# jmschrei/PyPore

Measured on AMD Instinct MI355X. Metric: Msamples/sec segmented (SpeedyStatSplit, 10^8-sample trace); %HBM roofline, higher is better.
Workload: dtype int32/f64 (exact integer block sums of fp32 or int16 samples; decisions in fp64)

## Files before the change

### pypore_amd/csrc/poreseg.hip

```cpp
#include <hip/hip_runtime.h>

#include <algorithm>
#include <atomic>
#include <chrono>
#include <complex>
#include <cmath>
#include <cstdarg>
#include <cstdio>
#include <cstdlib>
#include <cstring>
#include <initializer_list>
#include <condition_variable>
#include <mutex>
#include <string>
#include <thread>
#include <tuple>
#include <type_traits>
#include <vector>

#include "poreseg.h"
#include "seg_device.hpp"
#include "seg_align.hpp"
#include "seg_pairwise.hpp"
#include "seg_trf.hpp"
// ... 41 lines not shown

struct HostBuf : NoCopy {
    void *p = nullptr;
    size_t cap = 0;
    ~HostBuf() { release(); }
    hipError_t reserve(size_t bytes)
    {
        if (bytes <= cap) return hipSuccess;
        release();
        size_t want = std::max(bytes, cap + cap / 2);
        hipError_t e = hipHostMalloc(&p, want, hipHostMallocDefault);
        if (e == hipSuccess) { cap = want; g_live_bytes += cap; }
        return e;
    }
    void release() { if (p) { (void)hipHostFree(p); g_live_bytes -= cap; } p = nullptr; cap = 0; }
    template <class T> T *as() { return static_cast<T *>(p); }
};

struct Event : NoCopy {
    hipEvent_t e = nullptr;
    ~Event() { if (e) (void)hipEventDestroy(e); }
    operator hipEvent_t() const { return e; }
};

struct Stream : NoCopy {
    hipStream_t s = nullptr;
    bool own = false;
    ~Stream() { if (own && s) (void)hipStreamDestroy(s); }
    operator hipStream_t() const { return s; }
};

}

enum : int { SC_NO_LA = 1, SC_NO_UPLOAD = 2, SC_ALL = 3 };
constexpr int LA_KEEP = 16;
struct ps_ctx {
    int device = 0;
    int n_cu = 0;
    Stream stream;
    Event ev[10];
    Event ev_front[2];
    ~ps_ctx() { (void)hipSetDevice(device); if (stream.s) (void)hipStreamSynchronize(stream.s); }
    std::string err;
    int64_t tile_len = 0, halo = 0;
    int mode = MODE_FAST, spine_nt = 512, tree_nt = 256;
    int lds_max_samples = 0;
    int rep_eval = 1, rep_stage = 1, rep_sum = 1;
    uint8_t *d_is_spine = nullptr;
    int prune = 1;
    double wide_quantum = 0;
    int wide_skip = 0;
    int wide_mode = 0;
    int tree_mw = 0;
    int upload_by_kernel = 1;
    int k0_waves = 0;
    float noise_k = 0.1f;
    int k0_admit = 0;
    int k0_sets = 2;
    bool chain_held = false;
    unsigned long long chain_ticket = 0;
    bool defer_sync = false;
    int scan_lds_pad = 0;
    int k0_unaligned = 1;
    int single_pass = 1;
    int gather_fused = 1;
    int download_by_kernel = 1;
    int debug = 0;
// ... 36 lines not shown
        long long budget = 2ll << 30;
    } trf;
    DevBuf ev_info_tr;
    DevBuf blk_cls, cls_mm;
    DevBuf pre_c;
    struct { DevBuf tab, pre, tmp, stack, cnt, off; } ss;
    struct { DevBuf tab, tab2, mask, cnt, excl, off1, off2, hits, pair_off, keep, kept, y, len, span_off; } sp;
    struct {
        DevBuf log;
        int64_t cap = 65536, hdr_cap = -1;
        int64_t seen = -1, call_cap = 0;
        std::vector<int64_t> ev_start, ev_len;
    } nt;
    struct {
        DevBuf model, off, bp, last, flags;
        std::vector<char> blob;
        long long bp_budget = 512ll << 20;
        DevBuf fmat, acc, skip;
        DevBuf pmax;
        DevBuf samp;
        long long fb_budget = 4ll << 30;
        bool expect_lds = true;
    } hmm;
    int stitch_host = 0;
    DevBuf ev_len, det_counts, det_tics, det_cand;
    DevBuf bridges, bmeta, tile_i32, sp_off, spine_items, asm_hdr, ev_first_tile;
    DevBuf bridge_ext, ext_slot, ext_list;
    DevBuf lat_state, lat_seam, lat_res;
    unsigned lat_tag_next = 1;
    unsigned lat_tag_base = 0;
    int lat_help = 1;
    int bridge_budget = BR_MAX;
    int bridge_ext_on = 1;
    int short_chain = SC_ALL;
    int shared_n = 0;
    int hw_queues = 0;
    int pool_patience = BR_PATIENCE_POOL;
    int la_keep = 0;
    bool la_now = false;
    bool small_clean = false;
    bool small_clean_in = false;
    HostBuf h_hdr;
    DevBuf spine_jobs, spine_scratch, spine_dense, spine_meta, tree_jobs, tree_scratch, tree_spill, tree_defer, screen_acc,
        tree_counts, items, item_pos, first_item, ev_off, bounds_off, small;
    HostBuf h_meta, h_dense, h_small, h_up;
    int timing = 1;
    double ms[8] = {0, 0, 0, 0, 0, 0, 0, 0};
    int64_t counters[20] = {0, 0, 0, 0, 0, 0, 0, 0, 0, 0, 0, 0, 0, 0, -1, -1, 0, 0, 0, 0};
    bool screen_ran = false;
};

namespace {

int fail(ps_ctx *ctx, int code, const char *fmt, ...)
{
    if (ctx) {
        char buf[512];
        va_list ap;
        va_start(ap, fmt);
        vsnprintf(buf, sizeof buf, fmt, ap);
        va_end(ap);
        ctx->err = buf;
    }
    return code;
}

#define HIP_TRY(ctx, expr)                                                                        \
    do {                                                                                          \
        hipError_t e_ = (expr);                                                                   \
        if (e_ != hipSuccess)                                                                     \
            return fail(ctx, PS_ERR_HIP, "%s failed: %s (%s:%d)", #expr, hipGetErrorString(e_), __FILE__, __LINE__); \
    } while (0)

struct FrontStream { std::mutex mu; hipStream_t s = nullptr; };
FrontStream g_front[16];
FrontStream *front_for(ps_ctx *ctx)
{
    if (ctx->device < 0 || ctx->device >= 16) return nullptr;
    FrontStream *f = &g_front[ctx->device];
    std::lock_guard<std::mutex> lk(f->mu);
    if (!f->s) {
// ... 387 lines not shown
    return j;
}

int find_in(const TileList &t, int32_t pos)
{
    if (pos == t.start) return -1;
    auto it = std::lower_bound(t.a.begin(), t.a.end(), pos, [](const Anchor &x, int32_t v) { return x.pos < v; });
    if (it != t.a.end() && it->pos == pos) return static_cast<int>(it - t.a.begin());
    return -2;
}

}

namespace {
constexpr int RC_FALLBACK = 1;
constexpr int RC_WIDE = 2;
int finish_batch(ps_ctx *ctx, const DevCfg &cfg, size_t n_tj, int64_t n_items, int32_t n_ev,
                        int32_t *d_bounds, int64_t cap, int64_t *h_bounds_off, ps_segstat *d_stats,
                        std::chrono::steady_clock::time_point t_begin, const AsmHeader *d_hdr = nullptr,
                        AsmHeader *hdr_out = nullptr, bool wide_check = false)
{
    int rc;
    const size_t evb = (static_cast<size_t>(n_ev) + 1) * sizeof(int64_t);
    SmallLayout *sm = ctx->small.as<SmallLayout>();
    if (ctx->timing >= 2) HIP_TRY(ctx, hipEventRecord(ctx->ev[2], ctx->stream));
    if (n_tj) {
        const unsigned g = static_cast<unsigned>(std::min<size_t>(n_tj, 0x7fffffff));
        if (int lrc = launch_subtrees(ctx, cfg, g, sm, n_tj, d_hdr)) return lrc;
    }
    if (ctx->timing >= 2) HIP_TRY(ctx, hipEventRecord(ctx->ev[3], ctx->stream));
    const bool fused = d_hdr != nullptr && ctx->gather_fused;
    const bool one_copy = ctx->bounds_off.p == ctx->small.as<char>() + sizeof(SmallLayout);
    int dl_clear = 0;
    if (fused) {
        const int64_t blocks = (n_items >> GS_LOG) + 1;
        const unsigned gg = static_cast<unsigned>(std::max<int64_t>(1, std::min<int64_t>(blocks, 1024)));
        hipLaunchKernelGGL(gather_scan_kernel, dim3(gg), dim3(1 << GS_LOG), 0, ctx->stream, ctx->items.as<Item>(),
                           ctx->tree_jobs.as<TreeJob>(), ctx->tree_counts.as<int32_t>(), ctx->tree_scratch.as<int32_t>(),
                           static_cast<long long>(n_items), d_bounds, cap, ctx->d_is_spine, d_hdr, ctx->first_item.as<int64_t>(),
                           n_ev, ctx->bounds_off.as<int64_t>());
        HIP_TRY(ctx, hipGetLastError());
    } else {
    hipLaunchKernelGGL(item_scan_kernel, dim3(1), dim3(1024), 0, ctx->stream, ctx->items.as<Item>(),
                       ctx->tree_counts.as<int32_t>(), n_items, ctx->item_pos.as<int64_t>(), d_hdr,
                       ctx->first_item.as<int64_t>(), n_ev, ctx->bounds_off.as<int64_t>());
    HIP_TRY(ctx, hipGetLastError());
    }
    if (n_items && !fused) {
        const unsigned gg = static_cast<unsigned>(d_hdr ? std::min<int64_t>(n_items, 16384) : n_items);
        hipLaunchKernelGGL(gather_kernel, dim3(gg), dim3(64), 0, ctx->stream,
                           ctx->items.as<Item>(), ctx->tree_jobs.as<TreeJob>(), ctx->tree_counts.as<int32_t>(),
                           ctx->tree_scratch.as<int32_t>(), ctx->item_pos.as<int64_t>(), n_items, d_bounds, cap, ctx->d_is_spine,
                           d_hdr);
        HIP_TRY(ctx, hipGetLastError());
    }
    const bool stats_from_digest = d_stats != nullptr && cfg.bsum != nullptr && cfg.blk_mm != nullptr;
    if (stats_from_digest) {
        const int64_t scap = cap + n_ev;
        const unsigned sg = static_cast<unsigned>(std::min<int64_t>(std::max<int64_t>(scap, 1), 8192));
        by_dtype(cfg.dtype, [&](auto dt) {
            hipLaunchKernelGGL(segstat_bs_kernel<dt()>, dim3(sg), dim3(64), 0, ctx->stream, cfg, ctx->ev_off.as<int64_t>(),
                               ctx->ev_len.as<int64_t>(), n_ev, d_bounds, ctx->bounds_off.as<int64_t>(), d_stats, scap,
                               reinterpret_cast<unsigned *>(&sm->status), d_hdr);
        });
        HIP_TRY(ctx, hipGetLastError());
        if (ctx->timing >= 2) HIP_TRY(ctx, hipEventRecord(ctx->ev[4], ctx->stream));
    }
    if (one_copy) {
        HIP_TRY(ctx, ctx->h_small.reserve(sizeof(SmallLayout) + evb));
        void *h_dev = nullptr;
        if (ctx->download_by_kernel && hipHostGetDevicePointer(&h_dev, ctx->h_small.p, 0) != hipSuccess) { h_dev = nullptr; (void)hipGetLastError(); }
        if (h_dev) {
            static_assert(sizeof(SmallLayout) % 8 == 0, "the status block is copied in 8-byte words");
            const long long nw = static_cast<long long>((sizeof(SmallLayout) + evb) / 8);
            if (fused && d_stats == nullptr && ctx->screen_ran && (ctx->short_chain & SC_NO_UPLOAD)) dl_clear = static_cast<int>(sizeof(SmallLayout) / 8);
            hipLaunchKernelGGL(download_kernel, dim3(static_cast<unsigned>(std::min<long long>((nw + 255) / 256, 64))), dim3(256), 0, ctx->stream,
                               ctx->small.as<unsigned long long>(), static_cast<unsigned long long *>(h_dev), nw, dl_clear, &sm->hdr.fail);
            HIP_TRY(ctx, hipGetLastError());
        } else {
            HIP_TRY(ctx, hipMemcpyAsync(ctx->h_small.p, ctx->small.p, sizeof(SmallLayout) + evb, hipMemcpyDeviceToHost, ctx->stream));
        }
    } else {
        HIP_TRY(ctx, ctx->h_meta.reserve(evb));
        HIP_TRY(ctx, hipMemcpyAsync(ctx->h_meta.p, ctx->bounds_off.p, evb, hipMemcpyDeviceToHost, ctx->stream));
        HIP_TRY(ctx, hipMemcpyAsync(ctx->h_small.p, ctx->small.p, sizeof(SmallLayout), hipMemcpyDeviceToHost, ctx->stream));
    }
    if (ctx->timing >= 1) HIP_TRY(ctx, hipEventRecord(ctx->ev[9], ctx->stream));
    HIP_TRY(ctx, hipStreamSynchronize(ctx->stream));
    {
        float seq = 0;
        if (ctx->timing >= 1 && hipEventElapsedTime(&seq, ctx->ev[8], ctx->ev[9]) == hipSuccess) ctx->ms[7] = seq;
    }
    std::memcpy(h_bounds_off, one_copy ? ctx->h_small.as<char>() + sizeof(SmallLayout) : ctx->h_meta.as<char>(), evb);
    const SmallLayout hs = *ctx->h_small.as<SmallLayout>();
    if (wide_check && (static_cast<unsigned>(hs.status) & ST_WIDE_RANGE)) return RC_WIDE;
    rc = check_status(ctx, static_cast<unsigned>(hs.status));
    if (rc) return rc;
    if (d_hdr) {
        const AsmHeader hd = hs.hdr;
        if (hdr_out) *hdr_out = hd;
        if (hd.fail) {
            if (ctx->debug) {
                const size_t nt = static_cast<size_t>(ctx->counters[2]);
                std::vector<int4> bm(nt), mt(nt);
                std::vector<SpineJob> jb(nt);
                if (nt && hipMemcpy(bm.data(), ctx->bmeta.p, nt * sizeof(int4), hipMemcpyDeviceToHost) == hipSuccess &&
                    hipMemcpy(mt.data(), ctx->spine_meta.p, nt * sizeof(int4), hipMemcpyDeviceToHost) == hipSuccess &&
                    hipMemcpy(jb.data(), ctx->spine_jobs.p, nt * sizeof(SpineJob), hipMemcpyDeviceToHost) == hipSuccess) {
// ... 415 lines not shown
    if (front) {
        HIP_TRY(ctx, hipEventRecord(ctx->ev_front[1], fs));
        front_lock.unlock();
        HIP_TRY(ctx, hipStreamWaitEvent(ctx->stream, ctx->ev_front[1], 0));
    }
    if (nj) {
        const unsigned g = static_cast<unsigned>(nj);
        int lrc;
        if (wide) lrc = launch_scans_bs<DT_WIDE>(ctx, cfg, g, sm);
        else if (use_bs) lrc = launch_scans_bs<0>(ctx, cfg, g, sm);
        else {
            lrc = launch_spine_nt(ctx, cfg, g, sm, true);
            if (lrc) return lrc;
            if (ctx->timing >= 2) HIP_TRY(ctx, hipEventRecord(ctx->ev[6], ctx->stream));
            lrc = by_nt<256, 512>(ctx->spine_nt, [&](auto nt) {
                return by_dtype(cfg.dtype, [&](auto dt) { return launch_bridge<decltype(nt)::value, dt()>(ctx, cfg, g, sm); });
            });
        }
        if (lrc) return lrc;
    }
    if (ctx->timing >= 2) HIP_TRY(ctx, hipEventRecord(ctx->ev[1], ctx->stream));
    int *ti = ctx->tile_i32.as<int>();
    const size_t njp = std::max<size_t>(1, nj);
    const size_t tile_lds = (nj + 1) * sizeof(long long) + 4 * nj * sizeof(int);
    const int use_lds = tile_lds <= 150 * 1024;
    if (use_lds)
        HIP_TRY(ctx, set_dyn_lds(ctx, reinterpret_cast<const void *>(assemble_tiles_kernel), static_cast<int>(tile_lds)));
    AsmHeader hd = {};
    int rc = PS_OK;
    int64_t items_cap = max_items;
    int slots_used = 0, ext_stride = EXT_MAX;
    const bool no_la = nj && no_look_ahead(ctx, cfg);
    bool la_done = false, stride_set = false;
    for (int round = 0;; ++round) {
        hipLaunchKernelGGL(assemble_tiles_kernel, dim3(1), dim3(1024), use_lds ? tile_lds : 0, ctx->stream,
                           static_cast<int>(nj), ctx->spine_meta.as<int4>(), ctx->bmeta.as<int4>(),
                           ctx->ev_first_tile.as<int64_t>(), n_ev, ti, ti + njp, ti + 2 * njp, ti + 3 * njp,
                           ctx->sp_off.as<long long>(), ctx->first_item.as<int64_t>(), ctx->asm_hdr.as<AsmHeader>(),
                           static_cast<long long>(items_cap), use_lds, reinterpret_cast<const unsigned *>(&sm->status));
        HIP_TRY(ctx, hipGetLastError());
        const AsmHeader *d_hdr = ctx->asm_hdr.as<AsmHeader>();
        if (items_cap > 0) {
            const unsigned ag = static_cast<unsigned>(std::min<int64_t>((items_cap + 255) / 256, 2048));
            hipLaunchKernelGGL(assemble_items_kernel, dim3(ag), dim3(256), 0,
                               ctx->stream, ctx->spine_jobs.as<SpineJob>(), static_cast<int>(nj), ctx->spine_meta.as<int4>(),
                               ctx->spine_scratch.as<int2>(), ctx->bridges.as<int2>(), ti + 3 * njp,
                               ctx->sp_off.as<long long>(), static_cast<long long>(items_cap), mw, W, ctx->tree_jobs.as<TreeJob>(),
                               ctx->items.as<Item>(), ctx->tree_counts.as<int32_t>(), d_hdr, cfg.bsum != nullptr ? cfg.ev_info : nullptr,
                               ctx->bridge_ext.as<int2>(), ctx->ext_slot.as<int>(), ext_stride);
            HIP_TRY(ctx, hipGetLastError());
        }
        if (ctx->timing >= 2 && round == 0) HIP_TRY(ctx, hipEventRecord(ctx->ev[5], ctx->stream));
        rc = finish_batch(ctx, cfg, static_cast<size_t>(items_cap), items_cap, n_ev, d_bounds, cap, h_bounds_off, d_stats, t_begin,
                          d_hdr, &hd, use_bs);
        if (rc != RC_FALLBACK || !use_bs || !nj || round == EXT_ROUNDS + (la_done ? 1 : 0) || !ctx->bridge_ext_on) break;
        HIP_TRY(ctx, ctx->h_meta.reserve(2 * nj * sizeof(int4)));
        int4 *h_bm = ctx->h_meta.as<int4>(), *h_mt = h_bm + nj;
        HIP_TRY(ctx, hipMemcpyAsync(h_bm, ctx->bmeta.p, nj * sizeof(int4), hipMemcpyDeviceToHost, ctx->stream));
        HIP_TRY(ctx, hipMemcpyAsync(h_mt, ctx->spine_meta.p, nj * sizeof(int4), hipMemcpyDeviceToHost, ctx->stream));
        HIP_TRY(ctx, hipStreamSynchronize(ctx->stream));
        if (no_la && !la_done) {
            int64_t n_def = 0;
            for (size_t g = 0; g < nj; ++g) n_def += h_bm[g].w == BR_DEFER || h_bm[g].w == BR_DEFER_REACHED;
            if (n_def) {
                if (ctx->debug) fprintf(stderr, "[poreseg] look-ahead kernel behind the stitch: %lld deferred seams\n", static_cast<long long>(n_def));
                HIP_TRY(ctx, hipMemsetAsync(&sm->hdr, 0, sizeof(AsmHeader), ctx->stream));
                if (ctx->tree_screen) HIP_TRY(ctx, hipMemsetAsync(&sm->tree_defer[0], 0, sizeof sm->tree_defer[0], ctx->stream));
                if (int lrc = by_dtype(cfg.dtype, [&](auto dt) { return launch_bridge_la<dt()>(ctx, cfg, static_cast<unsigned>(nj), sm); })) return lrc;
                la_done = true;
                ctx->la_keep = LA_KEEP;
                ctx->counters[4] += n_def;
                ctx->counters[18] += n_def;
                continue;
            }
        }
        std::vector<int> list;
        bool hopeless = false;
        if (!stride_set) {
            size_t n_fail = 0;
            for (size_t g = 0; g < nj; ++g) n_fail += h_bm[g].w == BR_FAIL_REACHED || (h_bm[g].w == BR_FAIL && h_bm[g].x == ctx->bridge_budget);
            ext_stride = n_fail <= static_cast<size_t>(EXT_SLOTS) ? EXT_MAX : EXT_MAX_MANY;
            stride_set = true;
        }
// ... 228 lines not shown
    else if (n == "scan_bs") ctx->scan_bs = value != 0;
    else if (n == "near_tie_log" && value >= 0 && value <= (int64_t(1) << 30)) ctx->nt.cap = value;
    else if (n == "groups") ctx->groups = value != 0;
    else if (n == "tree_par") ctx->tree_par = value != 0;
    else if (n == "k0_waves" && value >= 0 && value <= 16) ctx->k0_waves = static_cast<int>(value);
    else if (n == "k0_shared") ctx->k0_shared = value != 0;
    else if (n == "k0_admit" && value >= 0) ctx->k0_admit = static_cast<int>(value);
    else if (n == "bridge_ext" && (value == 0 || value == 1)) ctx->bridge_ext_on = static_cast<int>(value);
    else if (n == "lat_help" && value >= 0 && value <= 2) ctx->lat_help = static_cast<int>(value);
    else if (n == "shared_device" && value >= 0 && value <= 4096) {
        ps_pool_plan_t plan;
        if (pool_plan(static_cast<int>(value), ctx->hw_queues > 0 ? ctx->hw_queues : process_hw_queues(), &plan) != PS_OK)
            return fail(ctx, PS_ERR_ARG, "shared_device: no plan for %lld contexts", static_cast<long long>(value));
        ctx->shared_n = static_cast<int>(value);
        ctx->la_keep = 0;
        ctx->k0_waves = plan.k0_waves;
        ctx->lat_help = plan.lat_help;
        ctx->k0_admit = plan.k0_admit;
    }
    else if (n == "hw_queues" && value >= 0 && value <= HW_QUEUES_MAX) ctx->hw_queues = static_cast<int>(value);
    else if (n == "hmm_bp_budget" && value >= 1) ctx->hmm.bp_budget = value;
    else if (n == "hmm_fb_budget" && value >= 1) ctx->hmm.fb_budget = value;
    else if (n == "pairwise_budget" && value >= 1) ctx->pw.budget = value;
    else if (n == "trf_budget" && value >= 1) ctx->trf.budget = value;
    else if (n == "hmm_expect_lds") ctx->hmm.expect_lds = value != 0;
    else if (n == "single_pass") ctx->single_pass = value != 0;
    else if (n == "gather_fused") ctx->gather_fused = value != 0;
    else if (n == "download_by_kernel") ctx->download_by_kernel = value != 0;
    else if (n == "debug") ctx->debug = value != 0;
    else if (n == "k0_unaligned") ctx->k0_unaligned = value != 0 ? k0_unaligned_probe(ctx->device, ctx->stream) : 0;
    else if (n == "slots_pct" && value >= 1 && value <= 100) ctx->slots_pct = static_cast<int>(value);
    else if (n == "tree_jobs_per_wave" && value >= 0 && value <= 1024) ctx->tree_jobs_per_wave = static_cast<int>(value);
    else if (n == "tree_screen") ctx->tree_screen = value != 0;
    else if (n == "short_chain" && value >= 0 && value <= 3) {
        static const int bits[4] = {0, SC_ALL, SC_NO_LA, SC_NO_UPLOAD};
        if (ctx->short_chain != bits[value]) ctx->small_clean = false;
        ctx->short_chain = bits[value];
    }
    else if (n == "bridge_patience" && value >= 1 && value <= 4096) { ctx->pool_patience = static_cast<int>(value); ctx->la_keep = 0; }
    else if (n == "noise_k_ppm" && value >= 0) ctx->noise_k = static_cast<float>(static_cast<double>(value) * 1.0e-6);
#ifdef PS_DIAG
    else if (n == "dbg_phase" && value >= 0 && value <= 2) ctx->dbg_phase = static_cast<int>(value);
    else if (n == "dbg_k0_nogrp") ctx->dbg_k0_nogrp = value != 0;
    else if (n == "cu_mask" && ctx->stream.own)
        return diag_mask_stream(ctx, &ctx->stream.s, static_cast<int>(value & 0xfff), static_cast<int>((value >> 12) & 0xfff),
                                static_cast<int>((value >> 24) & 0xff), ((value >> 32) & 1) != 0);
    else if (n == "k0_sets" && value >= 2 && value <= 4) ctx->k0_sets = static_cast<int>(value);
    else if (n == "scan_lds_pad" && value >= 0 && value <= 65536) ctx->scan_lds_pad = static_cast<int>(value);
    else if (n == "rep_eval" && value >= 1) ctx->rep_eval = static_cast<int>(value);
    else if (n == "rep_stage" && value >= 1) ctx->rep_stage = static_cast<int>(value);
    else if (n == "rep_sum" && value >= 1) ctx->rep_sum = static_cast<int>(value);
#endif
    else if (n == "bridge_budget" && value >= 1 && value <= BR_MAX) ctx->bridge_budget = static_cast<int>(value);
    else if (n == "wide_bs") { ctx->wide_bs = value != 0; ctx->wide_skip = 0; }
    else if (n == "bridge_single" && value >= 1) ctx->bridge_single = static_cast<int>(value);
    else if (n == "tree_tail_pct" && value >= 0 && value <= 100) ctx->tree_tail_pct = static_cast<int>(value);
    else if (n == "filter_fused") ctx->filt.fused = value != 0;
    else if (n == "upload_by_kernel") ctx->upload_by_kernel = value != 0;
    else if (n == "timing") ctx->timing = static_cast<int>(std::max<int64_t>(0, std::min<int64_t>(2, value)));
    else if (n == "tree_mw") ctx->tree_mw = value != 0;
    else if (n == "spine_nt" && (value == 256 || value == 512 || value == 1024)) ctx->spine_nt = static_cast<int>(value);
    else if (n == "tree_nt" && (value == 256 || value == 512)) ctx->tree_nt = static_cast<int>(value);
    else return fail(ctx, PS_ERR_ARG, "unknown option or value: %s", name);
    return PS_OK;
}

int ps_get_option(const ps_ctx *ctx, const char *name, int64_t *value)
{
// ... 828 lines not shown
    const int64_t *st = ctx->nt.ev_start.data(), *ln = ctx->nt.ev_len.data();
    const size_t ne = ctx->nt.ev_start.size();
    std::vector<int32_t> ord(ne);
    for (size_t e = 0; e < ne; ++e) ord[e] = static_cast<int32_t>(e);
    std::stable_sort(ord.begin(), ord.end(), [&](int32_t a, int32_t b) { return st[a] < st[b]; });
    std::vector<int64_t> reach(ne);
    for (size_t i = 0; i < ne; ++i) reach[i] = std::max(i ? reach[i - 1] : INT64_MIN, st[ord[i]] + ln[ord[i]]);
    std::vector<ps_near_tie> sites;
    for (const NtRec &r : rec) {
        const int64_t g = r.start, ge = r.start + r.len;
        size_t i = static_cast<size_t>(std::upper_bound(ord.begin(), ord.end(), g, [&](int64_t v, int32_t e) { return v < st[e]; }) - ord.begin());
        while (i > 0 && reach[i - 1] >= ge) {
            const int32_t e = ord[--i];
            if (st[e] <= g && ge <= st[e] + ln[e]) {
                const int32_t ws = static_cast<int32_t>(g - st[e]);
                sites.push_back({e, ws, static_cast<int32_t>(ge - st[e]), r.split < 0 ? -1 : ws + r.split});
            }
        }
    }
    auto key = [](const ps_near_tie &a) { return std::make_tuple(a.event, a.window_start, a.window_end, a.split); };
    std::sort(sites.begin(), sites.end(), [&](const ps_near_tie &a, const ps_near_tie &b) { return key(a) < key(b); });
    sites.erase(std::unique(sites.begin(), sites.end(), [&](const ps_near_tie &a, const ps_near_tie &b) { return key(a) == key(b); }),
                sites.end());
    *n_out = static_cast<int64_t>(sites.size());
    if (sites.size() > static_cast<size_t>(cap)) return PS_ERR_CAPACITY;
    std::copy(sites.begin(), sites.end(), out);
    return PS_OK;
}

int ps_get_timings(const ps_ctx *ctx, double *ms, int32_t n_ms, int64_t *counters, int32_t n_counters)
{
    if (!ctx) return PS_ERR_ARG;
    for (int i = 0; i < n_ms && ms; ++i) ms[i] = i < 8 ? ctx->ms[i] : 0.0;
    for (int i = 0; i < n_counters && counters; ++i) counters[i] = i < 20 ? ctx->counters[i] : 0;
    return PS_OK;
}

const int64_t *ps_counters(const ps_ctx *ctx) { return ctx ? ctx->counters : nullptr; }

int ps_synth_trace(ps_ctx *ctx, void *d_out, int32_t dtype, int64_t n, uint64_t seed,
                   const int64_t *h_seg_end, const int32_t *h_level_counts, int64_t nseg)
{
    if (!ctx) return PS_ERR_ARG;
    if (!d_out || n < 0 || nseg < 1 || !h_seg_end || !h_level_counts) return fail(ctx, PS_ERR_ARG, "bad argument");
    if (h_seg_end[nseg - 1] < n) return fail(ctx, PS_ERR_ARG, "segment table does not cover n");
    HIP_TRY(ctx, hipSetDevice(ctx->device));
    const size_t b1 = static_cast<size_t>(nseg) * sizeof(int64_t), b2 = static_cast<size_t>(nseg) * sizeof(int32_t);
    HIP_TRY(ctx, ctx->tree_scratch.reserve(b1 + b2));
    char *d = ctx->tree_scratch.as<char>();
    HIP_TRY(ctx, hipMemcpyAsync(d, h_seg_end, b1, hipMemcpyHostToDevice, ctx->stream));
    HIP_TRY(ctx, hipMemcpyAsync(d + b1, h_level_counts, b2, hipMemcpyHostToDevice, ctx->stream));
    HIP_TRY(ctx, hipStreamSynchronize(ctx->stream));
    hipLaunchKernelGGL(synth_kernel, dim3(4096), dim3(256), 0, ctx->stream, d_out, dtype, n,
                       static_cast<unsigned long long>(seed), reinterpret_cast<const int64_t *>(d),
                       reinterpret_cast<const int32_t *>(d + b1), nseg);
    HIP_TRY(ctx, hipGetLastError());
    HIP_TRY(ctx, hipStreamSynchronize(ctx->stream));
    return PS_OK;
}

namespace {
int filter_order_n(ps_ctx *ctx, const DevCfg &cfg, int64_t n, int order, double wn, double *d_out)
{
    typedef std::complex<double> cd;
    static const double poles[FILT_MAXORD + 1][4][2] = {
        {{0, 0}}, {{-0.9999999999999998, 0.0}},
        {{-0.8660254037844384, 0.4999999999999999}},
// ... 1352 lines not shown
```

### pypore_amd/csrc/seg_device.hpp

```cpp
#pragma once
#include <hip/hip_runtime.h>
#include <stdint.h>
#include "poreseg.h"

namespace ps {

constexpr int LDS_STACK = 128;
constexpr int MAX_WAVES = 16;
constexpr int OBUF = 256;
constexpr int BR_MAX = 256;
constexpr int LST_MAX = 256;
constexpr int LAT_D = 256;
constexpr int LAT_W = 16;
constexpr int LAT_C = 2048;
constexpr int LAT_TAGS = 4096;
struct LatHelp {
    unsigned long long *ctl;
    unsigned long long *state;
    int *seam;
    int *prog;
    unsigned long long *res;
    unsigned tag_base;
    int stay;
};
// ... 1908 lines not shown
        if (threadIdx.x == 1023) carry_s = base + run;
        __syncthreads();
    }
    if (threadIdx.x == 0) pos[n_items] = carry_s;
    __syncthreads();
    for (int e = threadIdx.x; e <= n_ev; e += 1024) bounds_off[e] = pos[first_item[e]];
}

__global__ __launch_bounds__(64) void gather_kernel(const Item *items, const TreeJob *jobs,
                                                    const int32_t *counts, const int32_t *scratch,
                                                    const int64_t *pos, int64_t n_items_host,
                                                    int32_t *bounds, int64_t cap, uint8_t *is_spine, const AsmHeader *hdr)
{
    const int64_t n_items = dev_count(hdr, n_items_host);
    for (int64_t it = blockIdx.x; it < n_items; it += gridDim.x) {
        const Item item = items[it];
        const int64_t p = pos[it];
        int cnt = 0;
        if (item.job >= 0) {
            cnt = counts[item.job];
            const int32_t *src = scratch + jobs[item.job].out_off;
            for (int i = threadIdx.x; i < cnt; i += 64)
                if (p + i < cap) { bounds[p + i] = src[i]; if (is_spine) is_spine[p + i] = 0; }
        }
        if (threadIdx.x == 0 && p + cnt < cap) { bounds[p + cnt] = item.anchor; if (is_spine) is_spine[p + cnt] = 1; }
    }
}



__global__ __launch_bounds__(256) void gather_scan_kernel(const Item *items, const TreeJob *jobs, const int32_t *counts,
                                                          const int32_t *scratch, long long n_items_host, int32_t *bounds,
                                                          int64_t cap, uint8_t *is_spine, const AsmHeader *hdr,
                                                          const int64_t *first_item, int32_t n_ev, int64_t *bounds_off)
{
    constexpr int GS = 1 << GS_LOG;
    __shared__ long long wsum[GS / 64];
    __shared__ int ws[GS / 64];
    __shared__ long long pos_s[GS];
    __shared__ int ev_lo_s, ev_hi_s;
    const bool failed = hdr && hdr->fail;
    const long long n_items = dev_count(hdr, n_items_host);
    const int32_t *blk = counts + n_items_host;
    const int tid = threadIdx.x, lane = tid & 63, wave = tid >> 6;
    if (failed) {
        for (long long e = blockIdx.x * static_cast<long long>(GS) + tid; e <= n_ev; e += gridDim.x * static_cast<long long>(GS)) bounds_off[e] = 0;
        return;
    }
    const long long nb = (n_items >> GS_LOG) + 1;
    for (long long b = blockIdx.x; b < nb; b += gridDim.x) {
        long long part = 0;
        for (long long k = tid; k < b; k += GS) part += blk[k];
#pragma unroll
        for (int d = 32; d >= 1; d >>= 1) part += __shfl_down(part, d);
        const long long i = (b << GS_LOG) + tid;
        const bool have = i < n_items;
        Item it = {-1, 0};
        int cnt = 0;
        if (have) { it = items[i]; if (it.job >= 0) cnt = counts[it.job]; }
        const int v = have ? cnt + 1 : 0;
        int inc = v;
#pragma unroll
        for (int d = 1; d < 64; d <<= 1) { const int u = __shfl_up(inc, d); if (lane >= d) inc += u; }
        if (lane == 0) wsum[wave] = part;
        if (lane == 63) ws[wave] = inc;
        if (tid < 2) {
            const long long key = (b + tid) << GS_LOG;
            int lo = 0, hi = n_ev + 1;
            while (lo < hi) { const int mid = (lo + hi) >> 1; if (first_item[mid] < key) lo = mid + 1; else hi = mid; }
            if (tid == 0) ev_lo_s = lo; else ev_hi_s = lo;
        }
        __syncthreads();
        long long p = (b << GS_LOG) + inc - v;
#pragma unroll
        for (int w = 0; w < GS / 64; ++w) { p += wsum[w]; if (w < wave) p += ws[w]; }
        pos_s[tid] = p;
        __syncthreads();
        for (int e = ev_lo_s + tid; e < ev_hi_s; e += GS) bounds_off[e] = pos_s[first_item[e] - (b << GS_LOG)];
        __syncthreads();
        const int32_t *src = cnt ? scratch + jobs[it.job].out_off : nullptr;
        unsigned long long big = __ballot(cnt > 16);
        while (big) {
            const int l = __builtin_ctzll(big);
            big &= big - 1ull;
            const long long pl = __shfl(p, l);
            const int cl = __shfl(cnt, l);
            const int32_t *sl = reinterpret_cast<const int32_t *>(__shfl(reinterpret_cast<unsigned long long>(src), l));
            for (int k = lane; k < cl; k += 64)
                if (pl + k < cap) { bounds[pl + k] = sl[k]; if (is_spine) is_spine[pl + k] = 0; }
        }
        if (cnt <= 16)
            for (int k = 0; k < cnt; ++k)
                if (p + k < cap) { bounds[p + k] = src[k]; if (is_spine) is_spine[p + k] = 0; }
        if (have && p + cnt < cap) { bounds[p + cnt] = it.anchor; if (is_spine) is_spine[p + cnt] = 1; }
    }
}

__global__ __launch_bounds__(256) void download_kernel(unsigned long long *src, unsigned long long *dst_host, long long n_words,
                                                       int clear_words = 0, const int *fail = nullptr)
{
    const long long nz = (clear_words > 0 && !(fail && *fail)) ? clear_words : 0;
    for (long long i = blockIdx.x * 256LL + threadIdx.x; i < n_words; i += gridDim.x * 256LL) {
        dst_host[i] = src[i];
        if (i < nz) src[i] = 0ull;
    }
}

__device__ __forceinline__ void chunk_exscan2(long long v1, long long v2, long long &e1, long long &e2,
                                              long long *wsum , long long *carry )
{
    const int lane = threadIdx.x & 63, wave = threadIdx.x >> 6;
// ... 62 lines not shown
        if (b.w == BR_FAIL || b.w == BR_DEFER || b.w == BR_FAIL_REACHED || b.w == BR_DEFER_REACHED) {
            fail_s = 1;
            if (b.w == BR_FAIL) bmeta[g].w = BR_FAIL_REACHED;
            if (b.w == BR_DEFER) bmeta[g].w = BR_DEFER_REACHED;
        }
    }
    __syncthreads();
    for (int g0 = 0; g0 < n_tiles; g0 += 1024) {
        const int g = g0 + tid;
        long long n = 0;
        if (g < n_tiles && reach[g]) {
            const int c = meta[g].x - entry[g];
            n = static_cast<long long>(c) + bmeta[g].x;
            if (c < 0) fail_s = 1;
        }
        long long e1, e2;
        chunk_exscan2(n, 0, e1, e2, wsum, carry);
        if (g < n_tiles) sp_off[g] = e1;
    }
    const long long n_items = carry[0];
    if (tid == 0) sp_off[n_tiles] = n_items;
    __syncthreads();
    for (int e = tid; e <= n_ev; e += 1024) first_item[e] = sp_off[ev_first_tile[e]];
    if (use_lds)
        for (int g = tid; g <= n_tiles; g += 1024) {
            sp_off_out[g] = sp_off[g];
            if (g < n_tiles) entry_out[g] = entry[g];
        }
    if (tid == 0) {
        hdr->n_items = n_items;
        hdr->n_jobs = n_items;
        hdr->tscratch = 0;
        hdr->fail = (fail_s || n_items > max_items) ? 1 : 0;
    }
}

__global__ __launch_bounds__(256) void assemble_items_kernel(
    const SpineJob *jobs, int n_tiles, const int4 *meta, const int2 *lists, const int2 *bridges,
    const int *entry, const long long *sp_off, long long n_items_host, int mw, int W,
    TreeJob *tjobs, Item *items, int32_t *counts, const AsmHeader *hdr, const int4 *ev_info,
    const int2 *ext = nullptr, const int *ext_slot = nullptr, int ext_stride = EXT_MAX)
{
    const long long n_items = dev_count(hdr, n_items_host);
    for (long long b = blockIdx.x * 256LL + threadIdx.x; b <= (n_items >> GS_LOG); b += gridDim.x * 256LL) counts[n_items_host + b] = 0;
    for (long long i = blockIdx.x * 256LL + threadIdx.x; i < n_items; i += gridDim.x * 256LL) {
    int lo = 0, hi = n_tiles - 1;
    while (lo < hi) {
        const int mid = (lo + hi) >> 1;
        if (sp_off[mid + 1] > i) hi = mid; else lo = mid + 1;
    }
    const int g = lo;
    const int k = static_cast<int>(i - sp_off[g]);
    const int en = entry[g], cnt = meta[g].x;
    const SpineJob jb2 = jobs[g];
    int2 el;
    int pred;
    if (k < cnt - en) {
        el = lists[jb2.out_off + en + k];
        pred = (en + k) > 0 ? lists[jb2.out_off + en + k - 1].x : jb2.start;
    } else {
        const int kb = k - (cnt - en);
        el = bridge_at(bridges, ext, ext_slot, ext_stride, g, kb);
        pred = kb > 0 ? bridge_at(bridges, ext, ext_slot, ext_stride, g, kb - 1).x : (cnt > 0 ? lists[jb2.out_off + cnt - 1].x : jb2.start);
    }
    const bool has = el.y == KIND_HIT || el.y == KIND_LATE;
    Item it;
    it.anchor = el.x;
    it.job = has ? static_cast<int32_t>(i) : -1;
    items[i] = it;
    TreeJob tj;
    tj.base = jb2.base;
    tj.start = pred;
    tj.end = el.x;
    tj.j0 = left_child_j0(pred, el.x, W, W / 2);
    tj.out_cap = has ? (el.x - pred) / mw + 1 : 0;
    tj.out_off = (jb2.vbase + pred) / mw + i;
    tj.pad_ = 0;
    if (ev_info) {
        const int4 info = ev_info[jb2.ev];
        tj.m = info.x;
        tj.pad_ = info.y;
        tj.boff = (static_cast<long long>(static_cast<unsigned>(info.w)) << 32) | static_cast<unsigned>(info.z);
    } else { tj.m = 0; tj.boff = 0; }
    tjobs[i] = tj;
    counts[i] = 0;
    }
}


constexpr int DET_NT = 256;
constexpr int DET_PER = 16;
constexpr int DET_CHUNK = DET_NT * DET_PER;

template <int DT>
__device__ __forceinline__ bool below_thr(const DevCfg &c, int k, double thr)
{
    return static_cast<double>(k) * c.q < thr;
}

template <int DT>
__global__ __launch_bounds__(DET_NT) void edge_scan_kernel(DevCfg c, int64_t n, double thr, int *tics,
                                                           unsigned *n_tics, unsigned tics_cap, int2 *chunk_mm,
                                                           unsigned *status)
{
    __shared__ int smin[DET_NT / 64], smax[DET_NT / 64];
    const int64_t i0 = static_cast<int64_t>(blockIdx.x) * DET_CHUNK + static_cast<int64_t>(threadIdx.x) * DET_PER;
    unsigned bits = 0, bad = 0;
    int mn = 0x7fffffff, mx = static_cast<int>(0x80000000);
    if (i0 < n) {
        int k[DET_PER];
        constexpr int ES = static_cast<int>(sizeof(typename Raw<DT>::type));
        const char *p = static_cast<const char *>(c.samples) + i0 * ES;
        if (i0 + DET_PER <= n && (reinterpret_cast<uintptr_t>(p) & 15u) == 0) {
            constexpr int NV = DET_PER * ES / 16;
            int4 raw[NV];
#pragma unroll
            for (int v = 0; v < NV; ++v) raw[v] = reinterpret_cast<const int4 *>(p)[v];
            if (sdt(DT) == PS_DTYPE_F32) {
#pragma unroll
// ... 280 lines not shown
```

### pypore_amd/engine.py

```python
import collections
import ctypes
import os
import threading
import warnings

import numpy as np
import torch

from . import _lib

_contexts = {}

DEFAULT_OPTIONS = {}
DEFAULT_TILING = [0, 0]
POOL_OVERRIDES = {}

EVENT_CAP = 1 << 16

_ENV_OPTIONS = {
    "PORESEG_MODE": "mode", "PORESEG_SPINE_NT": "spine_nt", "PORESEG_TREE_NT": "tree_nt", "PORESEG_PRUNE": "prune",
    "PORESEG_SCAN_BS": "scan_bs", "PORESEG_GROUPS": "groups", "PORESEG_TREE_PAR": "tree_par", "PORESEG_K0_WAVES": "k0_waves",
    "PORESEG_K0_SHARED": "k0_shared", "PORESEG_K0_MAX": "k0_admit", "PORESEG_K0_SETS": "k0_sets", "PORESEG_WIDE_BS": "wide_bs",
    "PORESEG_BRIDGE_SINGLE": "bridge_single", "PORESEG_TREE_TAIL": "tree_tail_pct", "PORESEG_FILTER_FUSED": "filter_fused",
    "PORESEG_UPLOAD": "upload_by_kernel", "PORESEG_TIMING": "timing", "PORESEG_TREE_MW": "tree_mw",
# ... 85 lines not shown
        if self.handle:
            self.L.ps_destroy(self.handle)
            self.handle = None

    def __del__(self):
        try:
            self.close()
        except Exception:
            pass

    def set_tiling(self, tile_len=0, halo=0):
        with self.lock:
            _lib.check(self.L.ps_set_tiling(self.handle, int(tile_len), int(halo)), self.handle)

    def set_option(self, name, value):
        with self.lock:
            _lib.check(self.L.ps_set_option(self.handle, name.encode(), int(value)), self.handle)

    def get_option(self, name):
        out = ctypes.c_int64()
        self.L.ps_get_option.argtypes = [ctypes.c_void_p, ctypes.c_char_p, ctypes.POINTER(ctypes.c_int64)]
        with self.lock:
            _lib.check(self.L.ps_get_option(self.handle, name.encode(), ctypes.byref(out)), self.handle)
        return int(out.value)

    def seq_ms(self):
        if not hasattr(self, "_tm"):
            self._tm = ((ctypes.c_double * 8)(), (ctypes.c_int64 * 8)())
        self.L.ps_get_timings(self.handle, self._tm[0], 8, self._tm[1], 8)
        return self._tm[0][7]

    def timings(self):
        ms = (ctypes.c_double * 8)()
        cnt = (ctypes.c_int64 * 20)()
        _lib.check(self.L.ps_get_timings(self.handle, ms, 8, cnt, 20))
        return dict(spine_ms=ms[0], tree_ms=ms[1], gather_ms=ms[2], total_ms=ms[3], stitch_ms=ms[4], bridge_ms=ms[5], blocksum_ms=ms[6], seq_ms=ms[7],
                    windows=cnt[0], candidates=cnt[1], tiles=cnt[2], tree_jobs=cnt[3], repairs=cnt[4],
                    exact_rescans=cnt[5], full_exact_scans=cnt[6], wide_redo=cnt[7],
                    windows_spine=cnt[8], windows_bridge=cnt[9], windows_tree=cnt[10], near_ties=cnt[11],
                    helper_chunks_published=cnt[12], helper_chunks_taken=cnt[13],
                    tree_deferred=cnt[14], windows_screen=cnt[15],
                    lookahead_skipped=cnt[16], upload_skipped=cnt[17], seams_resumed=cnt[18])

    def near_ties(self):
        if not hasattr(self, "_cnt"):
            self._cnt = self.L.ps_counters(self.handle)
        return int(self._cnt[11])

    def near_tie_sites(self):
        with self.lock:
            n = ctypes.c_int64()
            cap = 64
            while True:
                buf = (_lib.NearTie * cap)()
                rc = self.L.ps_get_near_ties(self.handle, buf, cap, ctypes.byref(n))
                if rc == _lib.PS_ERR_CAPACITY and n.value > cap:
                    cap = int(n.value)
                    continue
                _lib.check(rc, self.handle)
                break
            if n.value < 0:
                return None
            return np.frombuffer(buf, dtype=NEAR_TIE_DTYPE, count=int(n.value)).copy()

    @_serialised
    def segment_batch(self, samples, ev_off, params, quantum, offset_counts=0, want_stats=True, cap=None,
                      want_spine=False, lead=0, out=None, near_tie_warning=True):
        assert samples.is_cuda and samples.is_contiguous() and samples.dim() == 1
        if samples.dtype == torch.float32:
            dtype = _lib.PS_DTYPE_F32
        elif samples.dtype == torch.int16:
            dtype = _lib.PS_DTYPE_I16
        else:
            raise ValueError("samples must be float32 or int16, got %s" % samples.dtype)
        ev_off = np.ascontiguousarray(ev_off, dtype=np.int64)
# ... 952 lines not shown
```

Before: 600,800.

## Fuse tile assembly with item assembly and fold download into gather-scan kernel

Adds a single assemble_kernel that computes tile reachability, entry offsets and the item prefix scan in LDS and then builds items directly, replacing the separate assemble_tiles and assemble_items launches on the short route. It also lets gather_scan_kernel write the status block and bounds offsets straight to mapped host memory, so the separate download kernel can be skipped. Both are on by default via an expanded short_chain bitmask. The aim is to cut kernel launches and serialization on the latency-bound short chain. The cost is redundant per-block scan work, since every block of the grid recomputes the tile scan, and extra host-memory writes inside the gather kernel.

```diff
diff --git a/pypore_amd/csrc/poreseg.hip b/pypore_amd/csrc/poreseg.hip
--- a/pypore_amd/csrc/poreseg.hip
+++ b/pypore_amd/csrc/poreseg.hip
@@ -97,7 +97,10 @@
 
 }
 
-enum : int { SC_NO_LA = 1, SC_NO_UPLOAD = 2, SC_ALL = 3 };
+enum : int { SC_NO_LA = 1, SC_NO_UPLOAD = 2, SC_ONE_STITCH = 4, SC_NO_DOWNLOAD = 8, SC_ALL = 15 };
+#ifndef PS_SHORT_CHAIN
+#define PS_SHORT_CHAIN SC_ALL
+#endif
 constexpr int LA_KEEP = 16;
 struct ps_ctx {
     int device = 0;
@@ -200,7 +203,7 @@
     int lat_help = 1;
     int bridge_budget = BR_MAX;
     int bridge_ext_on = 1;
-    int short_chain = SC_ALL;
+    int short_chain = PS_SHORT_CHAIN;
     int shared_n = 0;
     int hw_queues = 0;
     int pool_patience = BR_PATIENCE_POOL;
@@ -214,7 +217,7 @@
     HostBuf h_meta, h_dense, h_small, h_up;
     int timing = 1;
     double ms[8] = {0, 0, 0, 0, 0, 0, 0, 0};
-    int64_t counters[20] = {0, 0, 0, 0, 0, 0, 0, 0, 0, 0, 0, 0, 0, 0, -1, -1, 0, 0, 0, 0};
+    int64_t counters[21] = {0, 0, 0, 0, 0, 0, 0, 0, 0, 0, 0, 0, 0, 0, -1, -1, 0, 0, 0, 0, 0};
     bool screen_ran = false;
 };
 
@@ -668,13 +671,25 @@
     const bool fused = d_hdr != nullptr && ctx->gather_fused;
     const bool one_copy = ctx->bounds_off.p == ctx->small.as<char>() + sizeof(SmallLayout);
     int dl_clear = 0;
+    void *h_dev = nullptr;
+    if (one_copy) {
+        HIP_TRY(ctx, ctx->h_small.reserve(sizeof(SmallLayout) + evb));
+        if (ctx->download_by_kernel && hipHostGetDevicePointer(&h_dev, ctx->h_small.p, 0) != hipSuccess) { h_dev = nullptr; (void)hipGetLastError(); }
+    }
+    static_assert(sizeof(SmallLayout) % 8 == 0 && offsetof(SmallLayout, hdr) % 8 == 0 && sizeof(AsmHeader) % 8 == 0, "the status block is copied in 8-byte words");
+    const bool plain_short = fused && h_dev && d_stats == nullptr && ctx->screen_ran;
+    if (plain_short && (ctx->short_chain & SC_NO_UPLOAD)) dl_clear = static_cast<int>(sizeof(SmallLayout) / 8);
+    const bool gather_copies = plain_short && (ctx->short_chain & SC_NO_DOWNLOAD);
     if (fused) {
         const int64_t blocks = (n_items >> GS_LOG) + 1;
         const unsigned gg = static_cast<unsigned>(std::max<int64_t>(1, std::min<int64_t>(blocks, 1024)));
         hipLaunchKernelGGL(gather_scan_kernel, dim3(gg), dim3(1 << GS_LOG), 0, ctx->stream, ctx->items.as<Item>(),
                            ctx->tree_jobs.as<TreeJob>(), ctx->tree_counts.as<int32_t>(), ctx->tree_scratch.as<int32_t>(),
                            static_cast<long long>(n_items), d_bounds, cap, ctx->d_is_spine, d_hdr, ctx->first_item.as<int64_t>(),
-                           n_ev, ctx->bounds_off.as<int64_t>());
+                           n_ev, ctx->bounds_off.as<int64_t>(),
+                           gather_copies ? ctx->small.as<unsigned long long>() : nullptr, gather_copies ? static_cast<unsigned long long *>(h_dev) : nullptr,
+                           static_cast<int>(sizeof(SmallLayout) / 8), static_cast<int>(offsetof(SmallLayout, hdr) / 8),
+                           static_cast<int>(sizeof(AsmHeader) / 8), dl_clear);
         HIP_TRY(ctx, hipGetLastError());
     } else {
     hipLaunchKernelGGL(item_scan_kernel, dim3(1), dim3(1024), 0, ctx->stream, ctx->items.as<Item>(),
@@ -703,13 +718,9 @@
         if (ctx->timing >= 2) HIP_TRY(ctx, hipEventRecord(ctx->ev[4], ctx->stream));
     }
     if (one_copy) {
-        HIP_TRY(ctx, ctx->h_small.reserve(sizeof(SmallLayout) + evb));
-        void *h_dev = nullptr;
-        if (ctx->download_by_kernel && hipHostGetDevicePointer(&h_dev, ctx->h_small.p, 0) != hipSuccess) { h_dev = nullptr; (void)hipGetLastError(); }
-        if (h_dev) {
-            static_assert(sizeof(SmallLayout) % 8 == 0, "the status block is copied in 8-byte words");
+        if (gather_copies) ctx->counters[20] += 1;
+        else if (h_dev) {
             const long long nw = static_cast<long long>((sizeof(SmallLayout) + evb) / 8);
-            if (fused && d_stats == nullptr && ctx->screen_ran && (ctx->short_chain & SC_NO_UPLOAD)) dl_clear = static_cast<int>(sizeof(SmallLayout) / 8);
             hipLaunchKernelGGL(download_kernel, dim3(static_cast<unsigned>(std::min<long long>((nw + 255) / 256, 64))), dim3(256), 0, ctx->stream,
                                ctx->small.as<unsigned long long>(), static_cast<unsigned long long *>(h_dev), nw, dl_clear, &sm->hdr.fail);
             HIP_TRY(ctx, hipGetLastError());
@@ -1191,14 +1202,28 @@
     int slots_used = 0, ext_stride = EXT_MAX;
     const bool no_la = nj && no_look_ahead(ctx, cfg);
     bool la_done = false, stride_set = false;
+    const bool one_stitch = (ctx->short_chain & SC_ONE_STITCH) != 0 && nj > 0 && nj <= static_cast<size_t>(ASM_MAX_TILES) &&
+                            max_items > 0 && max_items < 0x7fffffffLL && short_route(ctx, cfg);
     for (int round = 0;; ++round) {
+        const AsmHeader *d_hdr = ctx->asm_hdr.as<AsmHeader>();
+        if (one_stitch && round == 0) {
+            const unsigned ag = static_cast<unsigned>(std::min<int64_t>((items_cap + ASM_NT - 1) / ASM_NT, ASM_GRID));
+            hipLaunchKernelGGL(assemble_kernel, dim3(ag), dim3(ASM_NT), (3 * nj + 1) * sizeof(int), ctx->stream,
+                               ctx->spine_jobs.as<SpineJob>(), static_cast<int>(nj), ctx->spine_meta.as<int4>(), ctx->bmeta.as<int4>(),
+                               ctx->spine_scratch.as<int2>(), ctx->bridges.as<int2>(), ctx->ev_first_tile.as<int64_t>(), n_ev,
+                               ti + 3 * njp, ctx->sp_off.as<long long>(), ctx->first_item.as<int64_t>(), ctx->asm_hdr.as<AsmHeader>(),
+                               static_cast<long long>(items_cap), reinterpret_cast<const unsigned *>(&sm->status), mw, W,
+                               ctx->tree_jobs.as<TreeJob>(), ctx->items.as<Item>(), ctx->tree_counts.as<int32_t>(),
+                               cfg.bsum != nullptr ? cfg.ev_info : nullptr, ctx->bridge_ext.as<int2>(), ctx->ext_slot.as<int>(), ext_stride);
+            HIP_TRY(ctx, hipGetLastError());
+            ctx->counters[19] = 1;
+        } else {
         hipLaunchKernelGGL(assemble_tiles_kernel, dim3(1), dim3(1024), use_lds ? tile_lds : 0, ctx->stream,
                            static_cast<int>(nj), ctx->spine_meta.as<int4>(), ctx->bmeta.as<int4>(),
                            ctx->ev_first_tile.as<int64_t>(), n_ev, ti, ti + njp, ti + 2 * njp, ti + 3 * njp,
                            ctx->sp_off.as<long long>(), ctx->first_item.as<int64_t>(), ctx->asm_hdr.as<AsmHeader>(),
                            static_cast<long long>(items_cap), use_lds, reinterpret_cast<const unsigned *>(&sm->status));
         HIP_TRY(ctx, hipGetLastError());
-        const AsmHeader *d_hdr = ctx->asm_hdr.as<AsmHeader>();
         if (items_cap > 0) {
             const unsigned ag = static_cast<unsigned>(std::min<int64_t>((items_cap + 255) / 256, 2048));
             hipLaunchKernelGGL(assemble_items_kernel, dim3(ag), dim3(256), 0,
@@ -1208,6 +1233,7 @@
                                ctx->items.as<Item>(), ctx->tree_counts.as<int32_t>(), d_hdr, cfg.bsum != nullptr ? cfg.ev_info : nullptr,
                                ctx->bridge_ext.as<int2>(), ctx->ext_slot.as<int>(), ext_stride);
             HIP_TRY(ctx, hipGetLastError());
+        }
         }
         if (ctx->timing >= 2 && round == 0) HIP_TRY(ctx, hipEventRecord(ctx->ev[5], ctx->stream));
         rc = finish_batch(ctx, cfg, static_cast<size_t>(items_cap), items_cap, n_ev, d_bounds, cap, h_bounds_off, d_stats, t_begin,
@@ -1502,8 +1528,8 @@
     else if (n == "slots_pct" && value >= 1 && value <= 100) ctx->slots_pct = static_cast<int>(value);
     else if (n == "tree_jobs_per_wave" && value >= 0 && value <= 1024) ctx->tree_jobs_per_wave = static_cast<int>(value);
     else if (n == "tree_screen") ctx->tree_screen = value != 0;
-    else if (n == "short_chain" && value >= 0 && value <= 3) {
-        static const int bits[4] = {0, SC_ALL, SC_NO_LA, SC_NO_UPLOAD};
+    else if (n == "short_chain" && value >= 0 && value <= 5) {
+        static const int bits[6] = {0, SC_ALL, SC_NO_LA, SC_NO_UPLOAD, SC_NO_LA | SC_NO_UPLOAD | SC_ONE_STITCH, SC_NO_LA | SC_NO_UPLOAD | SC_NO_DOWNLOAD};
         if (ctx->short_chain != bits[value]) ctx->small_clean = false;
         ctx->short_chain = bits[value];
     }
@@ -2398,7 +2424,7 @@
 {
     if (!ctx) return PS_ERR_ARG;
     for (int i = 0; i < n_ms && ms; ++i) ms[i] = i < 8 ? ctx->ms[i] : 0.0;
-    for (int i = 0; i < n_counters && counters; ++i) counters[i] = i < 20 ? ctx->counters[i] : 0;
+    for (int i = 0; i < n_counters && counters; ++i) counters[i] = i < 21 ? ctx->counters[i] : 0;
     return PS_OK;
 }
 
diff --git a/pypore_amd/csrc/seg_device.hpp b/pypore_amd/csrc/seg_device.hpp
--- a/pypore_amd/csrc/seg_device.hpp
+++ b/pypore_amd/csrc/seg_device.hpp
@@ -1964,7 +1964,9 @@
 __global__ __launch_bounds__(256) void gather_scan_kernel(const Item *items, const TreeJob *jobs, const int32_t *counts,
                                                           const int32_t *scratch, long long n_items_host, int32_t *bounds,
                                                           int64_t cap, uint8_t *is_spine, const AsmHeader *hdr,
-                                                          const int64_t *first_item, int32_t n_ev, int64_t *bounds_off)
+                                                          const int64_t *first_item, int32_t n_ev, int64_t *bounds_off,
+                                                          unsigned long long *small = nullptr, unsigned long long *h_small = nullptr,
+                                                          int small_words = 0, int hdr_word = 0, int hdr_words = 0, int clear = 0)
 {
     constexpr int GS = 1 << GS_LOG;
     __shared__ long long wsum[GS / 64];
@@ -1975,8 +1977,19 @@
     const long long n_items = dev_count(hdr, n_items_host);
     const int32_t *blk = counts + n_items_host;
     const int tid = threadIdx.x, lane = tid & 63, wave = tid >> 6;
+    int64_t *h_off = h_small ? reinterpret_cast<int64_t *>(h_small + small_words) : nullptr;
+    if (h_small && blockIdx.x == 0) {
+        const bool zero = clear && !failed;
+        for (int w = tid; w < small_words; w += GS) {
+            h_small[w] = small[w];
+            if (zero && (w < hdr_word || w >= hdr_word + hdr_words)) small[w] = 0ull;
+        }
+    }
     if (failed) {
-        for (long long e = blockIdx.x * static_cast<long long>(GS) + tid; e <= n_ev; e += gridDim.x * static_cast<long long>(GS)) bounds_off[e] = 0;
+        for (long long e = blockIdx.x * static_cast<long long>(GS) + tid; e <= n_ev; e += gridDim.x * static_cast<long long>(GS)) {
+            bounds_off[e] = 0;
+            if (h_off) h_off[e] = 0;
+        }
         return;
     }
     const long long nb = (n_items >> GS_LOG) + 1;
@@ -2008,7 +2021,11 @@
         for (int w = 0; w < GS / 64; ++w) { p += wsum[w]; if (w < wave) p += ws[w]; }
         pos_s[tid] = p;
         __syncthreads();
-        for (int e = ev_lo_s + tid; e < ev_hi_s; e += GS) bounds_off[e] = pos_s[first_item[e] - (b << GS_LOG)];
+        for (int e = ev_lo_s + tid; e < ev_hi_s; e += GS) {
+            const long long pe = pos_s[first_item[e] - (b << GS_LOG)];
+            bounds_off[e] = pe;
+            if (h_off) h_off[e] = pe;
+        }
         __syncthreads();
         const int32_t *src = cnt ? scratch + jobs[it.job].out_off : nullptr;
         unsigned long long big = __ballot(cnt > 16);
@@ -2137,18 +2154,16 @@
         hdr->n_jobs = n_items;
         hdr->tscratch = 0;
         hdr->fail = (fail_s || n_items > max_items) ? 1 : 0;
-    }
-}
-
-__global__ __launch_bounds__(256) void assemble_items_kernel(
-    const SpineJob *jobs, int n_tiles, const int4 *meta, const int2 *lists, const int2 *bridges,
-    const int *entry, const long long *sp_off, long long n_items_host, int mw, int W,
-    TreeJob *tjobs, Item *items, int32_t *counts, const AsmHeader *hdr, const int4 *ev_info,
-    const int2 *ext = nullptr, const int *ext_slot = nullptr, int ext_stride = EXT_MAX)
-{
-    const long long n_items = dev_count(hdr, n_items_host);
-    for (long long b = blockIdx.x * 256LL + threadIdx.x; b <= (n_items >> GS_LOG); b += gridDim.x * 256LL) counts[n_items_host + b] = 0;
-    for (long long i = blockIdx.x * 256LL + threadIdx.x; i < n_items; i += gridDim.x * 256LL) {
+        hdr->pad = 0;
+    }
+}
+
+template <typename OffT>
+__device__ __forceinline__ void assemble_item(
+    long long i, const SpineJob *jobs, int n_tiles, const int4 *meta, const int2 *lists, const int2 *bridges,
+    const int *entry, const OffT *sp_off, int mw, int W, TreeJob *tjobs, Item *items, int32_t *counts, const int4 *ev_info,
+    const int2 *ext, const int *ext_slot, int ext_stride)
+{
     int lo = 0, hi = n_tiles - 1;
     while (lo < hi) {
         const int mid = (lo + hi) >> 1;
@@ -2189,7 +2204,117 @@
     } else { tj.m = 0; tj.boff = 0; }
     tjobs[i] = tj;
     counts[i] = 0;
-    }
+}
+
+__global__ __launch_bounds__(256) void assemble_items_kernel(
+    const SpineJob *jobs, int n_tiles, const int4 *meta, const int2 *lists, const int2 *bridges,
+    const int *entry, const long long *sp_off, long long n_items_host, int mw, int W,
+    TreeJob *tjobs, Item *items, int32_t *counts, const AsmHeader *hdr, const int4 *ev_info,
+    const int2 *ext = nullptr, const int *ext_slot = nullptr, int ext_stride = EXT_MAX)
+{
+    const long long n_items = dev_count(hdr, n_items_host);
+    for (long long b = blockIdx.x * 256LL + threadIdx.x; b <= (n_items >> GS_LOG); b += gridDim.x * 256LL) counts[n_items_host + b] = 0;
+    for (long long i = blockIdx.x * 256LL + threadIdx.x; i < n_items; i += gridDim.x * 256LL)
+        assemble_item(i, jobs, n_tiles, meta, lists, bridges, entry, sp_off, mw, W, tjobs, items, counts, ev_info, ext, ext_slot, ext_stride);
+}
+
+constexpr int ASM_NT = 256;
+constexpr int ASM_MAX_TILES = 4095;
+#ifndef PS_ASM_GRID
+#define PS_ASM_GRID 64
+#endif
+constexpr int ASM_GRID = PS_ASM_GRID;
+__global__ __launch_bounds__(ASM_NT) void assemble_kernel(
+    const SpineJob *jobs, int n_tiles, const int4 *meta, int4 *bmeta, const int2 *lists, const int2 *bridges,
+    const int64_t *ev_first_tile, int n_ev, int *entry_out, long long *sp_off_out, int64_t *first_item, AsmHeader *hdr,
+    long long max_items, const unsigned *status, int mw, int W, TreeJob *tjobs, Item *items, int32_t *counts,
+    const int4 *ev_info, const int2 *ext, const int *ext_slot, int ext_stride)
+{
+    extern __shared__ int asm_lds[];
+    __shared__ long long wsum[ASM_NT / 64];
+    __shared__ int fail_s;
+    const int tid = threadIdx.x, lane = tid & 63, wave = tid >> 6;
+    int *sp = asm_lds, *ja = sp + n_tiles + 1, *jb = ja + n_tiles;
+    long long n_items = 0;
+    int fail = 1;
+    if ((*status & ST_WIDE_RANGE) == 0u) {
+        if (tid == 0) fail_s = 0;
+        for (int g = tid; g < n_tiles; g += ASM_NT) {
+            sp[g] = 0;
+            const int4 b = bmeta[g];
+            ja[g] = b.w == BR_JOINED ? b.y : -1;
+        }
+        __syncthreads();
+        for (int e = tid; e < n_ev; e += ASM_NT)
+            if (ev_first_tile[e] < ev_first_tile[e + 1]) sp[ev_first_tile[e]] = 1;
+        __syncthreads();
+        int rounds = 1;
+        while ((1 << rounds) < n_tiles) ++rounds;
+        int *pa = ja, *pb = jb;
+        for (int r = 0; r <= rounds; ++r) {
+            for (int g = tid; g < n_tiles; g += ASM_NT) {
+                const int j = pa[g];
+                if (j >= 0 && sp[g]) sp[j] = 1;
+                pb[g] = j >= 0 ? pa[j] : -1;
+            }
+            __syncthreads();
+            int *t = pa; pa = pb; pb = t;
+        }
+        int *entry = jb;
+        for (int g = tid; g < n_tiles; g += ASM_NT) entry[g] = 0;
+        __syncthreads();
+        for (int g = tid; g < n_tiles; g += ASM_NT) {
+            if (!sp[g]) continue;
+            const int4 b = bmeta[g];
+            if (b.w == BR_JOINED) entry[b.y] = b.z + 1;
+            if (b.w == BR_FAIL || b.w == BR_DEFER || b.w == BR_FAIL_REACHED || b.w == BR_DEFER_REACHED) {
+                fail_s = 1;
+                if (blockIdx.x == 0) {
+                    if (b.w == BR_FAIL) bmeta[g].w = BR_FAIL_REACHED;
+                    if (b.w == BR_DEFER) bmeta[g].w = BR_DEFER_REACHED;
+                }
+            }
+        }
+        __syncthreads();
+        for (int g = tid; g < n_tiles; g += ASM_NT) {
+            int n = 0;
+            if (sp[g]) {
+                const int c = meta[g].x - entry[g];
+                n = c + bmeta[g].x;
+                if (c < 0) fail_s = 1;
+            }
+            ja[g] = n;
+        }
+        __syncthreads();
+        const int per = ((n_tiles + ASM_NT - 1) / ASM_NT) | 1;
+        const int g0 = min(tid * per, n_tiles), g1 = min(g0 + per, n_tiles);
+        long long tot = 0;
+        for (int g = g0; g < g1; ++g) tot += ja[g];
+        long long inc = tot;
+#pragma unroll
+        for (int d = 1; d < 64; d <<= 1) { const long long u = __shfl_up(inc, d); if (lane >= d) inc += u; }
+        if (lane == 63) wsum[wave] = inc;
+        __syncthreads();
+        long long run = inc - tot;
+        for (int w = 0; w < ASM_NT / 64; ++w) { n_items += wsum[w]; if (w < wave) run += wsum[w]; }
+        for (int g = g0; g < g1; ++g) { sp[g] = static_cast<int>(run); run += ja[g]; }
+        if (tid == 0) sp[n_tiles] = static_cast<int>(n_items);
+        __syncthreads();
+        fail = (fail_s || n_items > max_items) ? 1 : 0;
+        if (blockIdx.x == 0) {
+            for (int e = tid; e <= n_ev; e += ASM_NT) first_item[e] = sp[ev_first_tile[e]];
+            for (int g = tid; g <= n_tiles; g += ASM_NT) {
+                sp_off_out[g] = sp[g];
+                if (g < n_tiles) entry_out[g] = entry[g];
+            }
+        }
+    } else n_items = 0;
+    if (blockIdx.x == 0 && tid == 0) { hdr->n_items = n_items; hdr->n_jobs = n_items; hdr->tscratch = 0; hdr->fail = fail; hdr->pad = 0; }
+    if (fail) n_items = 0;
+    const long long n_items_host = max_items;
+    for (long long b = blockIdx.x * static_cast<long long>(ASM_NT) + tid; b <= (n_items >> GS_LOG); b += gridDim.x * static_cast<long long>(ASM_NT)) counts[n_items_host + b] = 0;
+    for (long long i = blockIdx.x * static_cast<long long>(ASM_NT) + tid; i < n_items; i += gridDim.x * static_cast<long long>(ASM_NT))
+        assemble_item(i, jobs, n_tiles, meta, lists, bridges, jb, sp, mw, W, tjobs, items, counts, ev_info, ext, ext_slot, ext_stride);
 }
 
 
diff --git a/pypore_amd/engine.py b/pypore_amd/engine.py
--- a/pypore_amd/engine.py
+++ b/pypore_amd/engine.py
@@ -141,15 +141,16 @@
 
     def timings(self):
         ms = (ctypes.c_double * 8)()
-        cnt = (ctypes.c_int64 * 20)()
-        _lib.check(self.L.ps_get_timings(self.handle, ms, 8, cnt, 20))
+        cnt = (ctypes.c_int64 * 21)()
+        _lib.check(self.L.ps_get_timings(self.handle, ms, 8, cnt, 21))
         return dict(spine_ms=ms[0], tree_ms=ms[1], gather_ms=ms[2], total_ms=ms[3], stitch_ms=ms[4], bridge_ms=ms[5], blocksum_ms=ms[6], seq_ms=ms[7],
                     windows=cnt[0], candidates=cnt[1], tiles=cnt[2], tree_jobs=cnt[3], repairs=cnt[4],
                     exact_rescans=cnt[5], full_exact_scans=cnt[6], wide_redo=cnt[7],
                     windows_spine=cnt[8], windows_bridge=cnt[9], windows_tree=cnt[10], near_ties=cnt[11],
                     helper_chunks_published=cnt[12], helper_chunks_taken=cnt[13],
                     tree_deferred=cnt[14], windows_screen=cnt[15],
-                    lookahead_skipped=cnt[16], upload_skipped=cnt[17], seams_resumed=cnt[18])
+                    lookahead_skipped=cnt[16], upload_skipped=cnt[17], seams_resumed=cnt[18],
+                    stitch_fused=cnt[19], download_skipped=cnt[20])
 
     def near_ties(self):
         if not hasattr(self, "_cnt"):
```

Result: no change. 601,400 (median of 2 runs) (+0.1%).
